# fricker2025-star/Tensor-Cuda-FFT-

Measured on AMD Instinct MI355X. Metric: spectral-mix fwd+bwd GSamples/s (B*N*D/s) at N=4096,D=256; %HBM roofline, higher is better.
Workload: dtype f32

## Files before the change

tensor-cuda-fft-_amd/csrc/smx_core.h:

```cpp
#pragma once
#include <stddef.h>
#include <stdint.h>

#if defined(__HIPCC__)
#include <hip/hip_runtime.h>
#define SMX_HD __host__ __device__ __forceinline__
#else
#define SMX_HD inline
#ifndef __restrict__
#define __restrict__ __restrict
#endif
struct float2 { float x, y; };
#endif

#ifndef SMX_NT_LOAD
#define SMX_NT_LOAD 1
#endif
#ifndef SMX_NT_STORE
#define SMX_NT_STORE 1
#endif

namespace smx {

#if defined(__HIPCC__)
// ... 514 lines not shown
template <int NB, int ROUND>
SMX_HD cf unpack_partner(const TState<NB>& st, const cf* __restrict__ U, int q, int qp, int j, int sl,
                         const ZSave<NB>& zs) {
  constexpr int S0 = ROUND * UnpackRounds<NB>::SLOTS;
  const int ps = partner_slot<NB>(q, sl);
  if (NB >= 4 && (sl & 15) == 0) {
    const bool own_bin = q == 0;
    const int pb = -band_beta(sl >> 4);
    const bool in_range = pb >= -(NB / 2) && pb < NB / 2;
    const cf own = zs.z[in_range ? band_index(pb) : (sl >> 4)];
    const cf u = U[(((own_bin ? sl : ps) - S0) * 16 + qp) * 16 + j];
    return own_bin ? own : u;
  }
  return U[((ps - S0) * 16 + qp) * 16 + j];
}

struct FilterArgs {
  const float* w_re;
  const float* w_im;
  const float* wt;
  const float* bias;
  float* xk_out;
  const float* xk_in;
  float* pslab;
  float* gb_part;
  int conj_w;
  const float* sc;
  float* gsc;
  cf* gsc_part;
  int goff, multi;
  float sp_scale;
  int sp_herm;
};
SMX_HD bool group_edge_slot(const FilterArgs& fa, int fs) {
  return (fa.multi && fs == -512) || (fa.goff > 0 && fs == 0);
}

constexpr int WL_PITCH = 34;
constexpr int WL_ELEMS = 128 * WL_PITCH;
struct WPre { float re[16], im[16]; };
SMX_HD void prefetch_w(WPre& w, const Geom& g, const float* __restrict__ w_re,
                       const float* __restrict__ w_im, int d0, int tid) {
  const int f = tid & 127, h = tid >> 7;
#pragma unroll
  for (int i = 0; i < 16; ++i) {
    const int d = d0 + h + 2 * i;
    const bool ok = d < g.D && f < g.k;
    const size_t o = ok ? (size_t)d * g.F + f : 0;
    const float a = w_re[o], b = w_im[o];
    w.re[i] = ok ? a : 0.f;
    w.im[i] = ok ? b : 0.f;
  }
}
SMX_HD void stage_w(const WPre& w, cf* __restrict__ wl, int tid, int conj_w) {
  const int f = tid & 127, h = tid >> 7;
#pragma unroll
  for (int i = 0; i < 16; ++i) wl[f * WL_PITCH + h + 2 * i] = mk(w.re[i], conj_w ? -w.im[i] : w.im[i]);
}

SMX_HD void synth_pair(const float (&r)[4], bool self, float scale, bool dbl, cf& Spos, cf& Sneg) {
  if (self) {
    Spos = mk(r[0] * scale, r[2] * scale);
    Sneg = Spos;
  } else {
    const float h = dbl ? scale : 0.5f * scale;
    Spos = mk((r[0] - r[3]) * h, (r[1] + r[2]) * h);
    Sneg = mk((r[0] + r[3]) * h, (-r[1] + r[2]) * h);
  }
}
template <int NB>
SMX_HD void synth_fill(TState<NB>& st, const Geom& g, const FilterArgs& fa, int b, int d, bool valid, int q) {
  const int dl = valid ? d : g.D - 2;
  constexpr int CH = NB == 8 ? 16 : 8;
#pragma unroll
  for (int c0 = 0; c0 < 16 * NB; c0 += CH) {
    float r[CH][4];
#pragma unroll
    for (int i = 0; i < CH; ++i) {
      const int fs = slot_fs<NB>(q, c0 + i);
      const int af = fs < 0 ? -fs : fs;
      const int afc = af < g.k ? af : 0;
      ld4(fa.xk_in + (((size_t)b * g.k + afc) * g.D + dl) * 2, r[i][0], r[i][1], r[i][2], r[i][3]);
    }
#pragma unroll
    for (int i = 0; i < CH; ++i) {
      const int fs = slot_fs<NB>(q, c0 + i);
      const int af = fs < 0 ? -fs : fs;
      const bool self = af == 0 || self_nyquist<NB>(g, fs);
      cf sp, sn;
      synth_pair(r[i], self, fa.sp_scale, fa.sp_herm && 2 * af != g.N, sp, sn);
      const cf S = (fs >= 0 || self) ? sp : sn;
      st.acc[c0 + i] = (valid && af < g.k) ? S : mk(0.f, 0.f);
    }
  }
}

template <int NB, int MODE, int ROUND = 0>
SMX_HD void unpack_phase2(TState<NB>& st, const cf* __restrict__ U, const Geom& g,
                          const FilterArgs& fa, int b, int d, bool valid, int q, int j,
                          const ZSave<NB>& zsave = ZSave<NB>{}, const cf* __restrict__ wl = nullptr,
                          cf* gs = nullptr) {
  const int qp = (16 - q) & 15;
  constexpr int S0 = ROUND * UnpackRounds<NB>::SLOTS;
  constexpr int NS = UnpackRounds<NB>::SLOTS;
#ifndef SMX_PF2_FWD
#define SMX_PF2_FWD 4
#endif
#ifndef SMX_PF2_BWD
#define SMX_PF2_BWD 8
#endif
  constexpr int PF = NB == 2 ? (MODE == 1 ? SMX_PF2_BWD : SMX_PF2_FWD) : NB >= 2 ? 4 : 0;
  constexpr bool XQ = MODE == 1 && !io_regs<NB, MODE>() && NB >= 2;
  float wq[PF ? PF : 1][4], xq[PF ? PF : 1][4];
  const int dl = valid ? d : g.D - 2;
  float sca = 1.f, scb = 1.f;
  if (fa.sc) { sca = fa.sc[(size_t)b * g.D + dl]; scb = fa.sc[(size_t)b * g.D + dl + 1]; }
  float gsx = 0.f, gsy = 0.f;
  auto issue = [&](int sl2, int ring) {
    const int fs2 = slot_fs<NB>(q, sl2);
    const int af2 = (fs2 < 0 ? -fs2 : fs2) + fa.goff;
    const int afc = af2 < g.k ? af2 : 0;
    if (MODE != 2) {
      if (fa.wt) {
        ld4(fa.wt + ((size_t)afc * g.D + dl) * 2, wq[ring][0], wq[ring][1], wq[ring][2], wq[ring][3]);
      } else {
        const size_t wo = (size_t)dl * g.F + afc;
        wq[ring][0] = fa.w_re[wo]; wq[ring][1] = fa.w_im[wo];
        wq[ring][2] = fa.w_re[wo + g.F]; wq[ring][3] = fa.w_im[wo + g.F];
      }
    }
    if (XQ && (slot_pos<NB>(sl2) || sl2 == 16 * (NB - 1)))
      ld4(fa.xk_in + (((size_t)b * g.k + afc) * g.D + dl) * 2, xq[ring][0], xq[ring][1], xq[ring][2],
          xq[ring][3]);
  };
  if (PF > 0) {
#pragma unroll
    for (int i = 0; i < PF && i < NS; ++i) issue(S0 + i, i);
  }
#pragma unroll
  for (int sl = S0; sl < S0 + UnpackRounds<NB>::SLOTS; ++sl) {
    const int fs = slot_fs<NB>(q, sl);
    const int af = (fs < 0 ? -fs : fs) + fa.goff;
    const bool snyq = self_nyquist<NB>(g, fs);
    const cf zo = st.acc[sl];
    const cf zp = unpack_partner<NB, ROUND>(st, U, q, qp, j, sl, zsave);
    const int ring = PF ? (sl - S0) % (PF ? PF : 1) : 0;
    float wv[4] = {0.f, 0.f, 0.f, 0.f}, xv[4] = {0.f, 0.f, 0.f, 0.f};
    if (PF > 0) {
#pragma unroll
      for (int c = 0; c < 4; ++c) { wv[c] = wq[ring][c]; xv[c] = xq[ring][c]; }
      if (sl + PF < S0 + NS) issue(sl + PF, ring);
    }
    const cf zpos = fs >= 0 ? zo : zp;
    const cf zneg = fs >= 0 ? zp : zo;
    const cf A = mk(0.5f * (zpos.x + zneg.x), 0.5f * (zpos.y - zneg.y));
    const cf Bc = mk(0.5f * (zpos.y + zneg.y), -0.5f * (zpos.x - zneg.x));
    cf S = mk(0.f, 0.f);
    if (valid && af < g.k && !(NB == 4 && group_edge_slot(fa, fs))) {
      cf wa = mk(0.f, 0.f), wb = mk(0.f, 0.f);
      if (MODE != 2) {
        if (NB == 1 && wl && af < 128) {
          float a0, a1, a2, a3;
          ld4(reinterpret_cast<const float*>(wl + af * WL_PITCH + 2 * j), a0, a1, a2, a3);
          wa = mk(a0, a1); wb = mk(a2, a3);
        } else {
          if (PF > 0) {
            wa = mk(wv[0], wv[1]); wb = mk(wv[2], wv[3]);
          } else if (fa.wt) {
            float a0, a1, a2, a3;
            ld4(fa.wt + ((size_t)af * g.D + d) * 2, a0, a1, a2, a3);
            wa = mk(a0, a1); wb = mk(a2, a3);
          } else {
            const size_t wo = (size_t)d * g.F + af;
            wa = mk(fa.w_re[wo], fa.w_im[wo]);
            wb = mk(fa.w_re[wo + g.F], fa.w_im[wo + g.F]);
          }
          if (fa.conj_w) { wa = cconj(wa); wb = cconj(wb); }
        }
        const cf ya = cscale(cmul(wa, A), sca), yb = cscale(cmul(wb, Bc), scb);
        if (af == 0 || snyq) {
          S = mk(ya.x * g.inv_n, yb.x * g.inv_n);
          if (MODE == 0 && fa.bias && af == 0) S = mk(S.x + fa.bias[d], S.y + fa.bias[d + 1]);
        } else if (fs > 0) {
          S = mk((ya.x - yb.y) * 0.5f * g.inv_n, (ya.y + yb.x) * 0.5f * g.inv_n);
        } else {
          S = mk((ya.x + yb.y) * 0.5f * g.inv_n, (-ya.y + yb.x) * 0.5f * g.inv_n);
        }
      }
      if (fs >= 0 || snyq) {
        const size_t xo = (((size_t)b * g.k + af) * g.D + d) * 2;
        if (io_regs<NB, MODE>() && !snyq) {
          constexpr int IM = io_bins<NB>() - 1;
          if (MODE != 1) {
// ... 103 lines not shown
        ld4(fa.xk_in + xo, xs[i][0], xs[i][1], xs[i][2], xs[i][3]);
      }
    }
#pragma unroll
    for (int i = 0; i < CH; ++i) {
      const int sl = c0 + i;
      const int fs = slot_fs<NB>(q, sl);
      const int af = (fs < 0 ? -fs : fs) + fa.goff;
      const bool ok = valid && af < g.k && !(NB == 4 && group_edge_slot(fa, fs));
      const bool snyq = self_nyquist<NB>(g, fs);
      const bool pos = slot_pos<NB>(sl) || snyq;
      const cf zo = st.acc[sl];
      const cf zpos = fs >= 0 ? zo : zp[i];
      const cf zneg = fs >= 0 ? zp[i] : zo;
      const cf A = mk(0.5f * (zpos.x + zneg.x), 0.5f * (zpos.y - zneg.y));
      const cf Bc = mk(0.5f * (zpos.y + zneg.y), -0.5f * (zpos.x - zneg.x));
      cf S = mk(0.f, 0.f);
      if (MODE != 2) {
        const cf wa = mk(war[i], cj ? -wai[i] : wai[i]);
        const cf wb = mk(wbr[i], cj ? -wbi[i] : wbi[i]);
        const cf ya = cscale(cmul(wa, A), sca), yb = cscale(cmul(wb, Bc), scb);
        const float h = 0.5f * g.inv_n;
        const cf sp = mk((ya.x - yb.y) * h, (ya.y + yb.x) * h);
        const cf sn = mk((ya.x + yb.y) * h, (-ya.y + yb.x) * h);
        cf s0 = mk(ya.x * g.inv_n, yb.x * g.inv_n);
        if (MODE == 0 && fa.bias && af == 0) s0 = mk(s0.x + fa.bias[dl], s0.y + fa.bias[dl + 1]);
        S = (af == 0 || snyq) ? s0 : (fs > 0 ? sp : sn);
        if (!ok) S = mk(0.f, 0.f);
      }
      st.acc[sl] = S;
      if (pos && ok) {
        const size_t xo = (((size_t)b * g.k + af) * g.D + d) * 2;
        if (MODE != 1) {
          if (fa.xk_out) st4(fa.xk_out + xo, A.x, A.y, Bc.x, Bc.y);
        } else {
          const cf pa = cscale(cmulc(mk(xs[i][0], xs[i][1]), A), g.inv_n);
          const cf pb = cscale(cmulc(mk(xs[i][2], xs[i][3]), Bc), g.inv_n);
          {
            const float wai_ = cj ? -wai[i] : wai[i], wbi_ = cj ? -wbi[i] : wbi[i];
            gsx += war[i] * pa.x + wai_ * pa.y; gsy += wbr[i] * pb.x + wbi_ * pb.y;
          }
          st4(fa.pslab + xo, pa.x * sca, pa.y * sca, pb.x * scb, pb.y * scb);
          if (af == 0) {
            fa.gb_part[(size_t)b * g.D + d] = A.x;
            fa.gb_part[(size_t)b * g.D + d + 1] = Bc.x;
          }
        }
      }
    }
  }
  if (MODE == 1 && gs) { gs->x += gsx; gs->y += gsy; }
}

}

namespace smx {

SMX_HD void fwd_phase2_out(const cf* __restrict__ E, const cf* __restrict__ bt_r, int t, int j,
                           cf* __restrict__ dst) {
  cf e[16];
#pragma unroll
  for (int t2 = 0; t2 < 16; ++t2) e[t2] = E[(t2 * 16 + t) * 16 + j];
  fft16<-1>(e);
#pragma unroll
  for (int s = 0; s < 16; ++s) dst[s * TPB] = cmul(ld_uniform(bt_r, s + BT_HALF), e[s]);
}
SMX_HD void inv_phase1_in(cf (&v)[16], const cf* __restrict__ bt_r, cf* __restrict__ E, int q, int j) {
#pragma unroll
  for (int s = 0; s < 16; ++s) v[s] = cmulc(v[s], ld_uniform(bt_r, s + BT_HALF));
  fft16<+1>(v);
#pragma unroll
  for (int p = 0; p < 16; ++p) E[(q * 16 + p) * 16 + j] = v[p];
}

template <int SGN, int L, int STRIDE = 256>
SMX_HD void fft_residues(cf (&a)[L], const cf* __restrict__ tw) {
  if constexpr (L == 8) {
    fft8<SGN>(a);
  } else if constexpr (L == 16) {
    fft16<SGN>(a);
  } else if constexpr (L > 16 && L % 2 == 0) {
    constexpr int H = L / 2;
    cf ev[H], od[H];
#pragma unroll
    for (int i = 0; i < H; ++i) { ev[i] = a[2 * i]; od[i] = a[2 * i + 1]; }
    fft_residues<SGN, H, 2 * STRIDE>(ev, tw);
    fft_residues<SGN, H, 2 * STRIDE>(od, tw);
#pragma unroll
    for (int k = 0; k < H; ++k) {
      const cf w = tw[STRIDE * k];
      const cf o = (SGN < 0) ? cmul(od[k], w) : cmulc(od[k], w);
      a[k] = cadd(ev[k], o);
      a[k + H] = csub(ev[k], o);
    }
  } else if constexpr (L == 4) {
    radix4<SGN>(a[0], a[1], a[2], a[3]);
  } else if constexpr (L == 2) {
    const cf s0 = cadd(a[0], a[1]), d0 = csub(a[0], a[1]);
    a[0] = s0; a[1] = d0;
  } else {
    cf o[L];
#pragma unroll
    for (int f2 = 0; f2 < L; ++f2) {
      cf acc = a[0];
#pragma unroll
      for (int r = 1; r < L; ++r) {
// ... 807 lines not shown
```

tensor-cuda-fft-_amd/csrc/smx_decim.hip:

```cpp
#include "smx_launch.h"

namespace smx {

template <int NB>
__device__ __forceinline__ void zero_acc(TState<NB>& st) {
#pragma unroll
  for (int s = 0; s < 16 * NB; ++s) st.acc[s] = mk(0.f, 0.f);
}

template <int NB, int MODE, bool BATCHED, int ROUND>
__device__ __forceinline__ void unpack_round(TState<NB>& st, cf* lds, const Geom& g,
                                             const FilterArgs& fa, int b, int d, bool valid, int t,
                                             int j, const ZSave<NB>& zs, const WPre* wp, cf* gs) {
  if constexpr (ROUND < UnpackRounds<NB>::N) {
    __syncthreads();
    unpack_phase1<NB, ROUND>(st, lds, t, j);
    const cf* wl = nullptr;
    if constexpr (NB == 1 && MODE != 2) {
      if (wp) { stage_w(*wp, lds + EX, t * 16 + j, fa.conj_w); wl = lds + EX; }
    }
    __syncthreads();
    if constexpr (BATCHED) unpack_phase2_batched<NB, MODE, ROUND>(st, lds, g, fa, b, d, valid, t, j, zs, gs, wl);
    else unpack_phase2<NB, MODE, ROUND>(st, lds, g, fa, b, d, valid, t, j, zs, wl, gs);
    unpack_round<NB, MODE, BATCHED, ROUND + 1>(st, lds, g, fa, b, d, valid, t, j, zs, wp, gs);
  }
}

template <int NB, int MODE, bool BATCHED>
__device__ __forceinline__ void unpack_filter(TState<NB>& st, cf* lds, const Geom& g,
                                              const FilterArgs& fa, int b, int d, bool valid, int t,
                                              int j, const WPre* wp = nullptr) {
  const ZSave<NB> zs = save_z<NB>(st);
  if constexpr (NB == 2 && MODE == 1 && !BATCHED) prefetch_io<NB, MODE>(st, g, fa, b, d, valid, t);
  cf gs = mk(0.f, 0.f);
  const bool want_gs = MODE == 1 && fa.gsc != nullptr;
  unpack_round<NB, MODE, BATCHED, 0>(st, lds, g, fa, b, d, valid, t, j, zs, wp, MODE == 1 ? &gs : nullptr);
  if constexpr (NB == 2 && MODE == 1 && !BATCHED) store_io<NB, MODE>(st, g, fa, b, d, valid, t);
  if constexpr (MODE == 1) {
    if (want_gs) {
      __syncthreads();
      lds[t * 16 + j] = gs;
      __syncthreads();
      if (t == 0 && valid) {
        float sa = 0.f, sb = 0.f;
#pragma unroll
        for (int u = 0; u < 16; ++u) { sa += lds[u * 16 + j].x; sb += lds[u * 16 + j].y; }
        fa.gsc[(size_t)b * g.D + d] = sa;
        fa.gsc[(size_t)b * g.D + d + 1] = sb;
      }
    }
  }
}

struct LnLoad {
  const cf* sb;
  float g0, g1, b0, b1;
};
template <int U0, int CNT>
__device__ __forceinline__ void load_stats(const cf* __restrict__ sb, const Geom& g, int t, int r,
                                           cf (&sv)[16]) {
  const cf* p = sb + (size_t)t * g.L + r;
#pragma unroll
  for (int u = U0; u < U0 + CNT; ++u) sv[u] = p[(size_t)u * 16 * g.L];
}

template <int NB, bool LN, bool DROP, bool PAD, bool LAST, class XB>
__device__ __forceinline__ void forward_tile(TState<NB>& st, cf* E, const XB& xb,
                                             const DecimArgs& a, int t, int j, int r, int rn, cf (&nx)[16],
                                             cf (&ns)[LN ? 16 : 1], const LnLoad* ln, Drop dr, unsigned pj) {
  const Geom& g = a.g;
  if constexpr (LN) {
#pragma unroll
    for (int u = 0; u < 16; ++u)
      st.v[u] = mk(fmaf((nx[u].x - ns[u].x) * ns[u].y, ln->g0, ln->b0),
                   fmaf((nx[u].y - ns[u].x) * ns[u].y, ln->g1, ln->b1));
  } else if constexpr (DROP) {
    const unsigned hd = (unsigned)(g.D >> 1), pstride = 16u * (unsigned)g.L * hd;
    const unsigned p0 = ((unsigned)t * (unsigned)g.L + (unsigned)r) * hd + pj;
#pragma unroll
    for (int u = 0; u < 16; ++u)
      st.v[u] = drop_apply(nx[u], drop_hash(p0 + (unsigned)u * pstride, dr.key), dr.thr, dr.scale);
  } else {
#pragma unroll
    for (int u = 0; u < 16; ++u) st.v[u] = nx[u];
  }
  if constexpr (!LAST) {
    load_rows<0, 8, PAD>(xb, rn, nx);
    if constexpr (LN) load_stats<0, 8>(ln->sb, g, t, rn, ns);
    __builtin_amdgcn_sched_barrier(0);
  }
  fwd_phase1_cp<NB>(st, E, t, j);
  if constexpr (!LAST) load_cp(a.tq + ((size_t)t * g.L + rn) * 16, st.cp);
  __syncthreads();
  if constexpr (!LAST) {
    load_rows<8, 8, PAD>(xb, rn, nx);
    if constexpr (LN) load_stats<8, 8>(ln->sb, g, t, rn, ns);
  }
  fwd_phase2<NB, true>(st, E, a.bt + (size_t)r * BT_STRIDE, t, j);
}

template <int NB, bool LN = false, bool DROP = false, bool PAD = false, class XB>
__device__ __forceinline__ void forward_loop(TState<NB>& st, cf* lds, const XB& xb,
                                             const DecimArgs& a, int t, int j, int rbeg, int cnt,
                                             int rot, const LnLoad* ln = nullptr, Drop dr = Drop{},
                                             unsigned pj = 0) {
  const Geom& g = a.g;
  const int rend = rbeg + cnt;
  cf nx[16];
  cf ns[LN ? 16 : 1];
  int r = rbeg + rot;
  load_rows<0, 16, PAD>(xb, r, nx);
  if constexpr (LN) load_stats<0, 16>(ln->sb, g, t, r, ns);
  load_cp(a.tq + ((size_t)t * g.L + r) * 16, st.cp);
  int i = 0;
  for (; i + 1 < cnt; ++i) {
    int rn = r + 1;
    if (rn == rend) rn = rbeg;
    forward_tile<NB, LN, DROP, PAD, false>(st, lds + (i & 1) * EX, xb, a, t, j, r, rn, nx, ns, ln, dr, pj);
    r = rn;
  }
  forward_tile<NB, LN, DROP, PAD, true>(st, lds + (i & 1) * EX, xb, a, t, j, r, r, nx, ns, ln, dr, pj);
}

template <int NB, bool RES, bool DROP, bool PAD, bool LAST, class YB, class RB>
__device__ __forceinline__ void inverse_tile(TState<NB>& st, cf* E, const YB& yb, const DecimArgs& a,
                                             int t, int j, int r, int rn,
                                             const RB& res, cf (&rx)[RES ? 16 : 1], Drop dr,
                                             unsigned pj, int sw) {
  const Geom& g = a.g;
  inv_phase1<NB, true>(st, a.bt + (size_t)r * BT_STRIDE, E, t, j);
  __syncthreads();
  inv_phase2_gather<NB>(st, E, t, j);
  if constexpr (!LAST) {
    __builtin_amdgcn_sched_barrier(0);
    load_cp(a.tq + ((size_t)t * g.L + rn) * 16, st.cp);
    __builtin_amdgcn_sched_barrier(0);
  }
  fft16<+1>(st.v);
  if constexpr (DROP) {
    const unsigned hd = (unsigned)(g.D >> 1), pstride = 16u * (unsigned)g.L * hd;
    const unsigned p0 = ((unsigned)t * (unsigned)g.L + (unsigned)r) * hd + pj;
#pragma unroll
    for (int u = 0; u < 16; ++u)
      st.v[u] = drop_apply(st.v[u], drop_hash(p0 + (unsigned)u * pstride, dr.key), dr.thr, dr.scale);
  }
  if constexpr (RES) {
#pragma unroll
    for (int u = 0; u < 16; ++u) st.v[u] = cadd(st.v[u], rx[u]);
    if constexpr (!LAST) load_rows<0, 16, PAD>(res, rn, rx);
  }
  store_rows<PAD>(yb, r, st.v, st_tile_mask(a, r, sw));
}

template <int NB, bool RES = false, bool DROP = false, bool PAD = false, class YB, class RB>
__device__ __forceinline__ void inverse_loop(TState<NB>& st, cf* lds, const YB& yb,
                                             const DecimArgs& a, int t, int j, int rbeg,
                                             int cnt, int rot, const RB& res, Drop dr = Drop{},
                                             unsigned pj = 0) {
  const Geom& g = a.g;
  int r = rbeg + rot;
  const int sw = (__builtin_amdgcn_readfirstlane(t) >> 2) >> a.st_wsh;
  cf rx[RES ? 16 : 1];
  if constexpr (RES) load_rows<0, 16, PAD>(res, r, rx);
  load_cp(a.tq + ((size_t)t * g.L + r) * 16, st.cp);
  __builtin_amdgcn_s_waitcnt(0x0F70);
  int i = 0;
  for (; i + 1 < cnt; ++i) {
    int rn = r + 1;
    if (rn == rbeg + cnt) rn = rbeg;
    inverse_tile<NB, RES, DROP, PAD, false>(st, lds + (i & 1) * EX, yb, a, t, j, r, rn, res, rx, dr, pj, sw);
    r = rn;
  }
  inverse_tile<NB, RES, DROP, PAD, true>(st, lds + (i & 1) * EX, yb, a, t, j, r, r, res, rx, dr, pj, sw);
}

__device__ __forceinline__ Drop make_drop(const DecimArgs& a, int b) {
  Drop dr;
  dr.thr = a.drop_thr; dr.scale = a.drop_scale;
  dr.key = drop_row_key(a.rng[0], a.rng[1], b);
  return dr;
}

constexpr bool fused_instance(int nb, int mode, bool drop, bool acc, bool pad, int io, int oio) {
  if (!among<1, 2, 4>::has(nb) || !among<0, 1, 2>::has(mode)) return false;
  if (acc) return nb == 4 && mode != 2 && !drop && io == 0 && oio == 0;
  if (io == 0) return oio == 0 && !(drop && (pad || mode == 2));
  return among<1, 2>::has(io) && mode != 2 && !pad && (oio == io || (oio == 0 && mode == 1));
}
template <int NB, int MODE, bool DROP = false, bool ACC = false, bool PAD = false, int IO = 0, int OIO = IO>
__global__ __launch_bounds__(TPB, 2) void k_fused(const DecimArgs a) {
  SMX_LDS_DECL;
  const Geom& g = a.g;
  const int tid = threadIdx.x, j = tid & 15, t = tid >> 4;
  const int ndt = (g.D + DT - 1) / DT;
  const WgItem w = wg_map(a.bid0 + blockIdx.x, g.B, ndt, 1, g.L, a.placement);
  const int b = w.b, d = w.dt * DT + 2 * j, rot = w.rot;
  const bool valid = d < g.D;
  RowBufT<IO> xb;
  if constexpr (IO == 0) xb = row_buf(a.in + (size_t)b * g.R * g.D, g, t, valid ? d : g.D - 2);
  else xb = row_buf<IO>(a.in, b, g, t, valid ? d : g.D - 2);

  TState<NB> st;
  zero_acc<NB>(st);
  if constexpr (NB == 1) prefetch_io<NB, MODE>(st, g, a.fa, b, d, valid, t);
  WPre wp;
  constexpr bool STAGE_W = NB == 1 && MODE != 2;
  if constexpr (STAGE_W) prefetch_w(wp, g, a.fa.w_re, a.fa.w_im, w.dt * DT, tid);
  Drop dr{};
  if constexpr (DROP) dr = make_drop(a, b);
  const unsigned pj = (unsigned)((valid ? d : g.D - 2) >> 1);
#ifndef SMX_AB_NO_FWD
  forward_loop<NB, false, DROP && MODE == 1, PAD>(st, lds, xb, a, t, j, 0, g.L, rot, nullptr, dr, pj);
#endif
#ifndef SMX_AB_NO_UNPACK
  unpack_filter<NB, MODE, false>(st, lds, g, a.fa, b, d, valid, t, j, STAGE_W ? &wp : nullptr);
#endif
#ifdef SMX_AB_NO_INV
  if (st.acc[0].x == 12345.f) a.out[0] = st.acc[1].y;
  return;
#endif
  if (a.out == nullptr) {
    if constexpr (NB == 1) store_io<NB, MODE>(st, g, a.fa, b, d, valid, t);
    if (a.ws_s != nullptr) {
      cf* s = a.ws_s + (size_t)(b * ndt + w.dt) * (16 * NB * TPB);
#pragma unroll
      for (int sl = 0; sl < 16 * NB; ++sl) s[sl * TPB + tid] = st.acc[sl];
    }
    return;
  }
  __syncthreads();
  RowBufT<OIO> yb;
  if constexpr (OIO == 0) yb = row_buf(a.out + (size_t)b * g.R * g.D, g, t, d, valid);
  else yb = row_buf<OIO>(a.out, b, g, t, d, valid);
  inverse_loop<NB, ACC, DROP && MODE == 0, PAD>(st, lds, yb, a, t, j, 0, g.L, rot, yb, dr, pj);
  if constexpr (NB == 1) store_io<NB, MODE>(st, g, a.fa, b, d, valid, t);
}

template <int NB, bool PAD, bool DROP>
__device__ __forceinline__ void forward16_loop(TState<NB>& st, cf* lds, const float* __restrict__ xb,
                                               const DecimArgs& a, int t, int j, int tbeg, int cnt, int rot,
                                               Drop dr, unsigned pj) {
  const Geom& g = a.g;
  const unsigned hd = (unsigned)(g.D >> 1);
  cf nx[16];
  int tau = tbeg + rot;
  load_tile16<PAD>(xb, g, t, tau, nx);
  cf cn = a.tw[min(16 * tau + t, g.N - 1)];
  for (int i = 0; i < cnt; ++i) {
    if constexpr (DROP) {
      const unsigned p0 = (unsigned)(16 * tau + t) * hd + pj, ps = (unsigned)g.P * hd;
#pragma unroll
      for (int u = 0; u < 16; ++u)
        st.v[u] = drop_apply(nx[u], drop_hash(p0 + (unsigned)u * ps, dr.key), dr.thr, dr.scale);
    } else {
#pragma unroll
      for (int u = 0; u < 16; ++u) st.v[u] = nx[u];
    }
    const cf c = cn;
    int tn = tau + 1;
    if (tn == tbeg + cnt) tn = tbeg;
    if (i + 1 < cnt) {
      load_tile16<PAD>(xb, g, t, tn, nx);
      cn = a.tw[min(16 * tn + t, g.N - 1)];
    }
    cf* E = lds + (i & 1) * EX;
    fwd_phase1<NB>(st, c, E, t, j);
    __syncthreads();
    fwd16_phase2<NB>(st, E, a.v16, a.b16 + (size_t)tau * 32, t, j);
    tau = tn;
  }
}
template <int NB, bool PAD, bool DROP>
__device__ __forceinline__ void inverse16_loop(TState<NB>& st, cf* lds, float* __restrict__ yb, const DecimArgs& a,
                                               int t, int j, bool valid, int tbeg, int cnt, int rot, Drop dr,
                                               unsigned pj) {
  const Geom& g = a.g;
  const unsigned hd = (unsigned)(g.D >> 1);
  int tau = tbeg + rot;
  for (int i = 0; i < cnt; ++i) {
    const cf c = a.tw[min(16 * tau + t, g.N - 1)];
    cf* E = lds + (i & 1) * EX;
    inv16_phase1<NB>(st, a.v16, a.b16 + (size_t)tau * 32, E, t, j);
    __syncthreads();
    inv_phase2<NB>(st, c, E, t, j);
    if constexpr (DROP) {
      const unsigned p0 = (unsigned)(16 * tau + t) * hd + pj, ps = (unsigned)g.P * hd;
#pragma unroll
      for (int u = 0; u < 16; ++u)
        st.v[u] = drop_apply(st.v[u], drop_hash(p0 + (unsigned)u * ps, dr.key), dr.thr, dr.scale);
    }
    store_tile16<PAD>(yb, g, t, tau, valid, st.v);
    ++tau;
    if (tau == tbeg + cnt) tau = tbeg;
  }
}

constexpr bool fused16_instance(int nb, int mode, bool pad, bool drop) {
  return among<1, 2>::has(nb) && among<0, 1, 2>::has(mode) && !(drop && (pad || mode == 2));
}
template <int NB, int MODE, bool PAD = false, bool DROP = false>
__global__ __launch_bounds__(TPB, 2) void k_fused16(const DecimArgs a) {
  SMX_LDS_DECL;
  const Geom& g = a.g;
  const int tid = threadIdx.x, j = tid & 15, t = tid >> 4;
  const int ndt = (g.D + DT - 1) / DT;
  const int T = g.L;
  const WgItem w = wg_map(a.bid0 + blockIdx.x, g.B, ndt, 1, T, a.placement);
  const int b = w.b, d = w.dt * DT + 2 * j, rot = w.rot;
  const bool valid = d < g.D;
  const float* xb = a.in + (size_t)b * g.R * g.D + (valid ? d : g.D - 2);
  TState<NB> st;
  zero_acc<NB>(st);
  if constexpr (NB == 1) prefetch_io<NB, MODE>(st, g, a.fa, b, d, valid, t);
  WPre wp;
  constexpr bool STAGE_W = NB == 1 && MODE != 2;
  if constexpr (STAGE_W) prefetch_w(wp, g, a.fa.w_re, a.fa.w_im, w.dt * DT, tid);
  Drop dr{};
  if constexpr (DROP) dr = make_drop(a, b);
  const unsigned pj = (unsigned)((valid ? d : g.D - 2) >> 1);
  forward16_loop<NB, PAD, DROP && MODE == 1>(st, lds, xb, a, t, j, 0, T, rot, dr, pj);
  unpack_filter<NB, MODE, false>(st, lds, g, a.fa, b, d, valid, t, j, STAGE_W ? &wp : nullptr);
  if (a.out == nullptr) {
    if constexpr (NB == 1) store_io<NB, MODE>(st, g, a.fa, b, d, valid, t);
    if (a.ws_s != nullptr) {
      cf* sp = a.ws_s + (size_t)(b * ndt + w.dt) * (16 * NB * TPB);
#pragma unroll
      for (int sl = 0; sl < 16 * NB; ++sl) sp[sl * TPB + tid] = st.acc[sl];
    }
    return;
  }
  __syncthreads();
  inverse16_loop<NB, PAD, DROP && MODE == 0>(st, lds, a.out + (size_t)b * g.R * g.D + d, a, t, j, valid, 0, T, rot, dr,
                                             pj);
  if constexpr (NB == 1) store_io<NB, MODE>(st, g, a.fa, b, d, valid, t);
}

constexpr bool split16_instance(int nb, bool pad, bool drop) {
  return among<1, 2>::has(nb) && !(pad && drop);
}
template <int NB, bool PAD = false, bool DROP = false>
__global__ __launch_bounds__(TPB, 2) void k_split16_a(const DecimArgs a) {
  SMX_LDS_DECL;
  const Geom& g = a.g;
  const int tid = threadIdx.x, j = tid & 15, t = tid >> 4;
  const int ndt = (g.D + DT - 1) / DT;
  const WgItem w = wg_map(a.bid0 + blockIdx.x, g.B, ndt, a.nsplit, a.lc, a.placement);
  const int c = w.c, b = w.b, wg = b * ndt + w.dt, d = w.dt * DT + 2 * j;
  const bool valid = d < g.D;
  const int tbeg = c * a.lc, cnt = min(a.lc, g.L - tbeg);
  const float* xb = a.in + (size_t)b * g.R * g.D + (valid ? d : g.D - 2);
  TState<NB> st;
  zero_acc<NB>(st);
  Drop dr{};
  if constexpr (DROP) dr = make_drop(a, b);
  if (cnt > 0)
    forward16_loop<NB, PAD, DROP>(st, lds, xb, a, t, j, tbeg, cnt, w.rot % cnt, dr,
                                  (unsigned)((valid ? d : g.D - 2) >> 1));
  cf* z = a.ws_z + ((size_t)wg * a.nsplit + c) * (16 * NB * TPB);
#pragma unroll
  for (int sl = 0; sl < 16 * NB; ++sl) z[sl * TPB + tid] = st.acc[sl];
}
template <int NB, bool PAD = false, bool DROP = false>
__global__ __launch_bounds__(TPB, 2) void k_split16_b(const DecimArgs a) {
  SMX_LDS_DECL;
  const Geom& g = a.g;
  const int tid = threadIdx.x, j = tid & 15, t = tid >> 4;
  const int ndt = (g.D + DT - 1) / DT;
  const WgItem w = wg_map(a.bid0 + blockIdx.x, g.B, ndt, a.nsplit, a.lc, a.placement);
  const int c = w.c, b = w.b, wg = b * ndt + w.dt, d = w.dt * DT + 2 * j;
  const bool valid = d < g.D;
  const int tbeg = c * a.lc, cnt = min(a.lc, g.L - tbeg);
  if (cnt <= 0) return;
  TState<NB> st;
  const cf* sp = a.ws_s + (size_t)wg * (16 * NB * TPB);
// ... 73 lines not shown

  TState<8> st;
  cf nx[16];
  load_tile<PAD>(xb, g, t, 0, nx);
  cf cn = a.tw[(size_t)t * 8];
  full8_fwd_tiles<0, MODE, PAD>(st, lds, xb, a, t, j, nx, cn);
  residue_fft8<-1>(st);
#ifndef SMX_FULL8_BATCHED
#define SMX_FULL8_BATCHED false
#endif
  unpack_filter<8, MODE, SMX_FULL8_BATCHED>(st, lds, g, a.fa, b, d, valid, t, j);
  if (a.out == nullptr) return;
  __syncthreads();
  residue_fft8<+1>(st);
  full8_inv_tiles<0, PAD>(st, lds, a.out + (size_t)b * g.R * g.D + d, a, t, j, valid);
}

template <bool PAD>
__global__ __launch_bounds__(TPB, 1) void k_synth8(const DecimArgs a) {
  SMX_LDS_DECL;
  const Geom& g = a.g;
  const int tid = threadIdx.x, j = tid & 15, t = tid >> 4;
  const int ndt = (g.D + DT - 1) / DT;
  const WgItem w = wg_map(a.bid0 + blockIdx.x, g.B, ndt, 1, g.L, a.placement);
  const int b = w.b, d = w.dt * DT + 2 * j;
  const bool valid = d < g.D;
  TState<8> st;
  synth_fill<8>(st, g, a.fa, b, d, valid, t);
  residue_fft8<+1>(st);
  full8_inv_tiles<0, PAD>(st, lds, a.out + (size_t)b * g.R * g.D + d, a, t, j, valid);
}

template <int NB, bool DROP = false, int IO = 0>
__global__ __launch_bounds__(TPB, NB > 2 ? 1 : 2) void k_fused_blk(const DecimArgs a) {
  SMX_LDS_DECL;
  const Geom& g = a.g;
  const int tid = threadIdx.x, j = tid & 15, t = tid >> 4;
  const int ndt = (g.D + DT - 1) / DT;
  const WgItem w = wg_map(a.bid0 + blockIdx.x, g.B, ndt, 1, g.L, a.placement);
  const int b = w.b, d = w.dt * DT + 2 * j, rot = w.rot;
  const bool valid = d < g.D;
  const int dc = valid ? d : g.D - 2;
  RowBufT<IO> xb;
  if constexpr (IO == 0) xb = row_buf(a.in + (size_t)b * g.R * g.D, g, t, dc);
  else xb = row_buf<IO>(a.in, b, g, t, dc);
  LnLoad ln;
  ln.sb = a.ln_stats + (size_t)b * g.N;
  ln.g0 = a.ln_w ? a.ln_w[dc] : 1.f; ln.g1 = a.ln_w ? a.ln_w[dc + 1] : 1.f;
  ln.b0 = a.ln_b ? a.ln_b[dc] : 0.f; ln.b1 = a.ln_b ? a.ln_b[dc + 1] : 0.f;

  TState<NB> st;
  zero_acc<NB>(st);
  WPre wp;
  if constexpr (NB == 1) prefetch_w(wp, g, a.fa.w_re, a.fa.w_im, w.dt * DT, tid);
  forward_loop<NB, true>(st, lds, xb, a, t, j, 0, g.L, rot, &ln);
  unpack_filter<NB, 0, false>(st, lds, g, a.fa, b, d, valid, t, j, NB == 1 ? &wp : nullptr);
  __syncthreads();
  RowBufT<IO> yb;
  if constexpr (IO == 0) yb = row_buf(a.out + (size_t)b * g.R * g.D, g, t, d, valid);
  else yb = row_buf<IO>(a.out, b, g, t, d, valid);
  Drop dr{};
  if constexpr (DROP) dr = make_drop(a, b);
  inverse_loop<NB, true, DROP>(st, lds, yb, a, t, j, 0, g.L, rot, xb, dr, (unsigned)(dc >> 1));
  if constexpr (NB == 1) store_io<NB, 0>(st, g, a.fa, b, d, valid, t);
}

constexpr bool split_a_instance(int nb, bool drop, bool pad, int io) {
  return among<1, 2, 4>::has(nb) && among<0, 1, 2>::has(io) && !(pad && (drop || io != 0));
}
template <int NB, bool DROP = false, bool PAD = false, int IO = 0>
__global__ __launch_bounds__(TPB, 2) void k_split_a(const DecimArgs a) {
  SMX_LDS_DECL;
  const Geom& g = a.g;
  const int tid = threadIdx.x, j = tid & 15, t = tid >> 4;
  const int ndt = (g.D + DT - 1) / DT;
  const WgItem w = wg_map(a.bid0 + blockIdx.x, g.B, ndt, a.nsplit, a.lc, a.placement);
  const int c = w.c, b = w.b, wg = b * ndt + w.dt, d = w.dt * DT + 2 * j;
  const bool valid = d < g.D;
  const int rbeg = c * a.lc, cnt = min(a.lc, g.L - rbeg);
  RowBufT<IO> xb;
  if constexpr (IO == 0) xb = row_buf(a.in + (size_t)b * g.R * g.D, g, t, valid ? d : g.D - 2);
  else xb = row_buf<IO>(a.in, b, g, t, valid ? d : g.D - 2);
  const int rot = w.rot % cnt;

  TState<NB> st;
  zero_acc<NB>(st);
  Drop dr{};
  if constexpr (DROP) dr = make_drop(a, b);
  forward_loop<NB, false, DROP, PAD>(st, lds, xb, a, t, j, rbeg, cnt, rot, nullptr, dr,
                                     (unsigned)((valid ? d : g.D - 2) >> 1));
  cf* z = a.ws_z + ((size_t)wg * a.nsplit + c) * (16 * NB * TPB);
#pragma unroll
  for (int sl = 0; sl < 16 * NB; ++sl) z[sl * TPB + tid] = st.acc[sl];
}

template <int NB>
__global__ __launch_bounds__(TPB) void k_split_sum(const DecimArgs a) {
  const int sl = blockIdx.x % (16 * NB), wg = blockIdx.x / (16 * NB), tid = threadIdx.x;
  const cf* z = a.ws_z + (size_t)wg * a.nsplit * (16 * NB * TPB) + sl * TPB + tid;
  cf acc = mk(0.f, 0.f);
  int c = 0;
  for (; c + 8 <= a.nsplit; c += 8) {
    cf v[8];
#pragma unroll
    for (int u = 0; u < 8; ++u) v[u] = z[(size_t)(c + u) * (16 * NB * TPB)];
#pragma unroll
    for (int u = 0; u < 8; ++u) acc = cadd(acc, v[u]);
  }
  for (; c < a.nsplit; ++c) acc = cadd(acc, z[(size_t)c * (16 * NB * TPB)]);
  a.ws_zs[(size_t)wg * (16 * NB * TPB) + sl * TPB + tid] = acc;
}

template <int NB, int MODE>
__global__ __launch_bounds__(TPB, NB > 1 ? 1 : 2) void k_split_f(const DecimArgs a) {
  SMX_LDS_DECL;
  const Geom& g = a.g;
// ... 220 lines not shown
```

Before: 339.4.

## Add staged unpack path for NB=1 and carry twiddle state across phases

```diff
diff --git a/tensor-cuda-fft-_amd/csrc/smx_core.h b/tensor-cuda-fft-_amd/csrc/smx_core.h
--- a/tensor-cuda-fft-_amd/csrc/smx_core.h
+++ b/tensor-cuda-fft-_amd/csrc/smx_core.h
@@ -590,6 +590,10 @@
     w.im[i] = ok ? b : 0.f;
   }
 }
+SMX_HD cf prefetch_bias(const Geom& g, const float* __restrict__ bias, int d, bool valid) {
+  const int dl = valid ? d : g.D - 2;
+  return bias ? mk(bias[dl], bias[dl + 1]) : mk(0.f, 0.f);
+}
 SMX_HD void stage_w(const WPre& w, cf* __restrict__ wl, int tid, int conj_w) {
   const int f = tid & 127, h = tid >> 7;
 #pragma unroll
@@ -633,14 +637,15 @@
   }
 }
 
-template <int NB, int MODE, int ROUND = 0>
+template <int NB, int MODE, int ROUND = 0, int SL0 = ROUND * UnpackRounds<NB>::SLOTS,
+          int SL1 = SL0 + UnpackRounds<NB>::SLOTS>
 SMX_HD void unpack_phase2(TState<NB>& st, const cf* __restrict__ U, const Geom& g,
                           const FilterArgs& fa, int b, int d, bool valid, int q, int j,
                           const ZSave<NB>& zsave = ZSave<NB>{}, const cf* __restrict__ wl = nullptr,
                           cf* gs = nullptr) {
   const int qp = (16 - q) & 15;
-  constexpr int S0 = ROUND * UnpackRounds<NB>::SLOTS;
-  constexpr int NS = UnpackRounds<NB>::SLOTS;
+  constexpr int S0 = SL0;
+  constexpr int NS = SL1 - SL0;
 #ifndef SMX_PF2_FWD
 #define SMX_PF2_FWD 4
 #endif
@@ -676,7 +681,7 @@
     for (int i = 0; i < PF && i < NS; ++i) issue(S0 + i, i);
   }
 #pragma unroll
-  for (int sl = S0; sl < S0 + UnpackRounds<NB>::SLOTS; ++sl) {
+  for (int sl = S0; sl < S0 + NS; ++sl) {
     const int fs = slot_fs<NB>(q, sl);
     const int af = (fs < 0 ? -fs : fs) + fa.goff;
     const bool snyq = self_nyquist<NB>(g, fs);
@@ -886,6 +891,98 @@
   if (MODE == 1 && gs) { gs->x += gsx; gs->y += gsy; }
 }
 
+SMX_HD constexpr bool packed_sums_fused(int sl) { return (sl >= 1 && sl <= 4) || (sl >= 8 && sl <= 12); }
+SMX_HD float rounded(float x) {
+#if defined(__HIP_DEVICE_COMPILE__)
+  asm("" : "+v"(x));
+#endif
+  return x;
+}
+SMX_HD cf packed_sums(bool fused, bool pos, cf ca, cf cb, cf ya, cf yb, float sca, float scb) {
+#if defined(__HIP_DEVICE_COMPILE__)
+  if (fused)
+    return pos ? mk(__builtin_fmaf(-scb, cb.y, ya.x), __builtin_fmaf(sca, ca.y, yb.x))
+               : mk(__builtin_fmaf(scb, cb.y, ya.x), __builtin_fmaf(-sca, ca.y, yb.x));
+#endif
+  (void)fused; (void)ca; (void)cb; (void)sca; (void)scb;
+  const float yax = rounded(ya.x), yay = rounded(ya.y), ybx = rounded(yb.x), yby = rounded(yb.y);
+  return pos ? mk(yax - yby, yay + ybx) : mk(yax + yby, -yay + ybx);
+}
+
+template <int MODE>
+SMX_HD void unpack_phase2_staged(TState<1>& st, const cf* __restrict__ U, const Geom& g, const FilterArgs& fa,
+                                 int b, int d, bool valid, int q, int j, const cf* __restrict__ wl, cf bias,
+                                 cf* gs = nullptr) {
+  static_assert(MODE == 0 || MODE == 1, "the spectrum-only launches read no filter");
+  const int qp = (16 - q) & 15;
+  const int dl = valid ? d : g.D - 2;
+  const ZSave<1> zs{};
+  float sca = 1.f, scb = 1.f;
+  if (fa.sc) { sca = fa.sc[(size_t)b * g.D + dl]; scb = fa.sc[(size_t)b * g.D + dl + 1]; }
+  const bool add_bias = MODE == 0 && fa.bias != nullptr;
+  const cf z8 = st.acc[8];
+  cf zp[16];
+  float w[16][4];
+#pragma unroll
+  for (int sl = 0; sl < 16; ++sl) {
+    const int fs = slot_fs<1>(q, sl);
+    const int af = fs < 0 ? -fs : fs;
+    const int afc = (af < g.k && af < 128) ? af : 0;
+    zp[sl] = unpack_partner<1, 0>(st, U, q, qp, j, sl, zs);
+    ld4(reinterpret_cast<const float*>(wl + afc * WL_PITCH + 2 * j), w[sl][0], w[sl][1], w[sl][2], w[sl][3]);
+  }
+  float gsx = 0.f, gsy = 0.f;
+  cf A0 = mk(0.f, 0.f), B0 = mk(0.f, 0.f);
+#pragma unroll
+  for (int sl = 0; sl < 16; ++sl) {
+    const bool pos = sl < 8;
+    const int fs = slot_fs<1>(q, sl);
+    const int af = fs < 0 ? -fs : fs;
+    const bool ok = valid && af < g.k && af < 128;
+    const cf zo = st.acc[sl];
+    const cf zpos = pos ? zo : zp[sl];
+    const cf zneg = pos ? zp[sl] : zo;
+    const cf A = mk(0.5f * (zpos.x + zneg.x), 0.5f * (zpos.y - zneg.y));
+    const cf Bc = mk(0.5f * (zpos.y + zneg.y), -0.5f * (zpos.x - zneg.x));
+    const cf wa = mk(w[sl][0], w[sl][1]), wb = mk(w[sl][2], w[sl][3]);
+    const cf ca = cmul(wa, A), cb = cmul(wb, Bc);
+    const cf ya = cscale(ca, sca), yb = cscale(cb, scb);
+    const cf ps = packed_sums(packed_sums_fused(sl), pos, ca, cb, ya, yb, sca, scb);
+    cf S = mk(ps.x * 0.5f * g.inv_n, ps.y * 0.5f * g.inv_n);
+    if (sl == 0) {
+      cf s0 = mk(rounded(ya.x * g.inv_n), rounded(yb.x * g.inv_n));
+      const cf s0b = mk(s0.x + bias.x, s0.y + bias.y);
+      s0 = add_bias ? s0b : s0;
+      S = af == 0 ? s0 : S;
+      A0 = A; B0 = Bc;
+    }
+    st.acc[sl] = ok ? S : mk(0.f, 0.f);
+    if (pos) {
+      cf& ia = st.io[2 * sl];
+      cf& ib = st.io[2 * sl + 1];
+      if (MODE == 0) {
+        ia = ok ? A : ia; ib = ok ? Bc : ib;
+      } else {
+        const cf pa = cscale(cmulc(ia, A), g.inv_n);
+        const cf pb = cscale(cmulc(ib, Bc), g.inv_n);
+        const float tx = wa.x * pa.x + wa.y * pa.y, ty = wb.x * pb.x + wb.y * pb.y;
+        gsx = ok ? gsx + tx : gsx; gsy = ok ? gsy + ty : gsy;
+        const cf oa = cscale(pa, sca), ob = cscale(pb, scb);
+        ia = ok ? oa : ia; ib = ok ? ob : ib;
+      }
+    }
+  }
+  if (MODE == 1 && q == 0 && valid && g.k > 0) {
+    fa.gb_part[(size_t)b * g.D + d] = A0.x;
+    fa.gb_part[(size_t)b * g.D + d + 1] = B0.x;
+  }
+  if (MODE == 1 && gs) { gs->x += gsx; gs->y += gsy; }
+  if (g.k > 128) {
+    st.acc[8] = z8;
+    unpack_phase2<1, MODE, 0, 8, 9>(st, U, g, fa, b, d, valid, q, j, zs, wl, gs);
+  }
+}
+
 }
 
 namespace smx {
diff --git a/tensor-cuda-fft-_amd/csrc/smx_decim.hip b/tensor-cuda-fft-_amd/csrc/smx_decim.hip
--- a/tensor-cuda-fft-_amd/csrc/smx_decim.hip
+++ b/tensor-cuda-fft-_amd/csrc/smx_decim.hip
@@ -1,6 +1,10 @@
 #include "smx_launch.h"
 
 namespace smx {
+
+#ifndef SMX_CARRY_CP
+#define SMX_CARRY_CP true
+#endif
 
 template <int NB>
 __device__ __forceinline__ void zero_acc(TState<NB>& st) {
@@ -11,7 +15,7 @@
 template <int NB, int MODE, bool BATCHED, int ROUND>
 __device__ __forceinline__ void unpack_round(TState<NB>& st, cf* lds, const Geom& g,
                                              const FilterArgs& fa, int b, int d, bool valid, int t,
-                                             int j, const ZSave<NB>& zs, const WPre* wp, cf* gs) {
+                                             int j, const ZSave<NB>& zs, const WPre* wp, cf bias, cf* gs) {
   if constexpr (ROUND < UnpackRounds<NB>::N) {
     __syncthreads();
     unpack_phase1<NB, ROUND>(st, lds, t, j);
@@ -20,21 +24,28 @@
       if (wp) { stage_w(*wp, lds + EX, t * 16 + j, fa.conj_w); wl = lds + EX; }
     }
     __syncthreads();
+#ifdef SMX_AB_UNPACK_SLOTS
+    constexpr bool STAGED = false;
+#else
+    constexpr bool STAGED = NB == 1 && MODE != 2 && !BATCHED;
+#endif
     if constexpr (BATCHED) unpack_phase2_batched<NB, MODE, ROUND>(st, lds, g, fa, b, d, valid, t, j, zs, gs, wl);
+    else if constexpr (STAGED)
+      unpack_phase2_staged<MODE>(st, lds, g, fa, b, d, valid, t, j, wl, bias, gs);
     else unpack_phase2<NB, MODE, ROUND>(st, lds, g, fa, b, d, valid, t, j, zs, wl, gs);
-    unpack_round<NB, MODE, BATCHED, ROUND + 1>(st, lds, g, fa, b, d, valid, t, j, zs, wp, gs);
+    unpack_round<NB, MODE, BATCHED, ROUND + 1>(st, lds, g, fa, b, d, valid, t, j, zs, wp, bias, gs);
   }
 }
 
 template <int NB, int MODE, bool BATCHED>
 __device__ __forceinline__ void unpack_filter(TState<NB>& st, cf* lds, const Geom& g,
                                               const FilterArgs& fa, int b, int d, bool valid, int t,
-                                              int j, const WPre* wp = nullptr) {
+                                              int j, const WPre* wp = nullptr, cf bias = mk(0.f, 0.f)) {
   const ZSave<NB> zs = save_z<NB>(st);
   if constexpr (NB == 2 && MODE == 1 && !BATCHED) prefetch_io<NB, MODE>(st, g, fa, b, d, valid, t);
   cf gs = mk(0.f, 0.f);
   const bool want_gs = MODE == 1 && fa.gsc != nullptr;
-  unpack_round<NB, MODE, BATCHED, 0>(st, lds, g, fa, b, d, valid, t, j, zs, wp, MODE == 1 ? &gs : nullptr);
+  unpack_round<NB, MODE, BATCHED, 0>(st, lds, g, fa, b, d, valid, t, j, zs, wp, bias, MODE == 1 ? &gs : nullptr);
   if constexpr (NB == 2 && MODE == 1 && !BATCHED) store_io<NB, MODE>(st, g, fa, b, d, valid, t);
   if constexpr (MODE == 1) {
     if (want_gs) {
@@ -64,7 +75,7 @@
   for (int u = U0; u < U0 + CNT; ++u) sv[u] = p[(size_t)u * 16 * g.L];
 }
 
-template <int NB, bool LN, bool DROP, bool PAD, bool LAST, class XB>
+template <int NB, bool LN, bool DROP, bool PAD, bool LAST, bool CARRY, class XB>
 __device__ __forceinline__ void forward_tile(TState<NB>& st, cf* E, const XB& xb,
                                              const DecimArgs& a, int t, int j, int r, int rn, cf (&nx)[16],
                                              cf (&ns)[LN ? 16 : 1], const LnLoad* ln, Drop dr, unsigned pj) {
@@ -90,7 +101,7 @@
     __builtin_amdgcn_sched_barrier(0);
   }
   fwd_phase1_cp<NB>(st, E, t, j);
-  if constexpr (!LAST) load_cp(a.tq + ((size_t)t * g.L + rn) * 16, st.cp);
+  if constexpr (!LAST || CARRY) load_cp(a.tq + ((size_t)t * g.L + rn) * 16, st.cp);
   __syncthreads();
   if constexpr (!LAST) {
     load_rows<8, 8, PAD>(xb, rn, nx);
@@ -99,7 +110,7 @@
   fwd_phase2<NB, true>(st, E, a.bt + (size_t)r * BT_STRIDE, t, j);
 }
 
-template <int NB, bool LN = false, bool DROP = false, bool PAD = false, class XB>
+template <int NB, bool LN = false, bool DROP = false, bool PAD = false, bool CARRY = false, class XB>
 __device__ __forceinline__ void forward_loop(TState<NB>& st, cf* lds, const XB& xb,
                                              const DecimArgs& a, int t, int j, int rbeg, int cnt,
                                              int rot, const LnLoad* ln = nullptr, Drop dr = Drop{},
@@ -116,10 +127,10 @@
   for (; i + 1 < cnt; ++i) {
     int rn = r + 1;
     if (rn == rend) rn = rbeg;
-    forward_tile<NB, LN, DROP, PAD, false>(st, lds + (i & 1) * EX, xb, a, t, j, r, rn, nx, ns, ln, dr, pj);
+    forward_tile<NB, LN, DROP, PAD, false, false>(st, lds + (i & 1) * EX, xb, a, t, j, r, rn, nx, ns, ln, dr, pj);
     r = rn;
   }
-  forward_tile<NB, LN, DROP, PAD, true>(st, lds + (i & 1) * EX, xb, a, t, j, r, r, nx, ns, ln, dr, pj);
+  forward_tile<NB, LN, DROP, PAD, true, CARRY>(st, lds + (i & 1) * EX, xb, a, t, j, r, rbeg + rot, nx, ns, ln, dr, pj);
 }
 
 template <int NB, bool RES, bool DROP, bool PAD, bool LAST, class YB, class RB>
@@ -152,7 +163,7 @@
   store_rows<PAD>(yb, r, st.v, st_tile_mask(a, r, sw));
 }
 
-template <int NB, bool RES = false, bool DROP = false, bool PAD = false, class YB, class RB>
+template <int NB, bool RES = false, bool DROP = false, bool PAD = false, bool CARRIED = false, class YB, class RB>
 __device__ __forceinline__ void inverse_loop(TState<NB>& st, cf* lds, const YB& yb,
                                              const DecimArgs& a, int t, int j, int rbeg,
                                              int cnt, int rot, const RB& res, Drop dr = Drop{},
@@ -162,7 +173,7 @@
   const int sw = (__builtin_amdgcn_readfirstlane(t) >> 2) >> a.st_wsh;
   cf rx[RES ? 16 : 1];
   if constexpr (RES) load_rows<0, 16, PAD>(res, r, rx);
-  load_cp(a.tq + ((size_t)t * g.L + r) * 16, st.cp);
+  if constexpr (!CARRIED) load_cp(a.tq + ((size_t)t * g.L + r) * 16, st.cp);
   __builtin_amdgcn_s_waitcnt(0x0F70);
   int i = 0;
   for (; i + 1 < cnt; ++i) {
@@ -206,14 +217,17 @@
   WPre wp;
   constexpr bool STAGE_W = NB == 1 && MODE != 2;
   if constexpr (STAGE_W) prefetch_w(wp, g, a.fa.w_re, a.fa.w_im, w.dt * DT, tid);
+  cf bias = mk(0.f, 0.f);
+  if constexpr (STAGE_W && MODE == 0) bias = prefetch_bias(g, a.fa.bias, d, valid);
   Drop dr{};
   if constexpr (DROP) dr = make_drop(a, b);
   const unsigned pj = (unsigned)((valid ? d : g.D - 2) >> 1);
+  constexpr bool CARRY = SMX_CARRY_CP && MODE == 0 && !ACC;
 #ifndef SMX_AB_NO_FWD
-  forward_loop<NB, false, DROP && MODE == 1, PAD>(st, lds, xb, a, t, j, 0, g.L, rot, nullptr, dr, pj);
+  forward_loop<NB, false, DROP && MODE == 1, PAD, CARRY>(st, lds, xb, a, t, j, 0, g.L, rot, nullptr, dr, pj);
 #endif
 #ifndef SMX_AB_NO_UNPACK
-  unpack_filter<NB, MODE, false>(st, lds, g, a.fa, b, d, valid, t, j, STAGE_W ? &wp : nullptr);
+  unpack_filter<NB, MODE, false>(st, lds, g, a.fa, b, d, valid, t, j, STAGE_W ? &wp : nullptr, bias);
 #endif
 #ifdef SMX_AB_NO_INV
   if (st.acc[0].x == 12345.f) a.out[0] = st.acc[1].y;
@@ -232,7 +246,7 @@
   RowBufT<OIO> yb;
   if constexpr (OIO == 0) yb = row_buf(a.out + (size_t)b * g.R * g.D, g, t, d, valid);
   else yb = row_buf<OIO>(a.out, b, g, t, d, valid);
-  inverse_loop<NB, ACC, DROP && MODE == 0, PAD>(st, lds, yb, a, t, j, 0, g.L, rot, yb, dr, pj);
+  inverse_loop<NB, ACC, DROP && MODE == 0, PAD, CARRY>(st, lds, yb, a, t, j, 0, g.L, rot, yb, dr, pj);
   if constexpr (NB == 1) store_io<NB, MODE>(st, g, a.fa, b, d, valid, t);
 }
 
@@ -315,11 +329,13 @@
   WPre wp;
   constexpr bool STAGE_W = NB == 1 && MODE != 2;
   if constexpr (STAGE_W) prefetch_w(wp, g, a.fa.w_re, a.fa.w_im, w.dt * DT, tid);
+  cf bias = mk(0.f, 0.f);
+  if constexpr (STAGE_W && MODE == 0) bias = prefetch_bias(g, a.fa.bias, d, valid);
   Drop dr{};
   if constexpr (DROP) dr = make_drop(a, b);
   const unsigned pj = (unsigned)((valid ? d : g.D - 2) >> 1);
   forward16_loop<NB, PAD, DROP && MODE == 1>(st, lds, xb, a, t, j, 0, T, rot, dr, pj);
-  unpack_filter<NB, MODE, false>(st, lds, g, a.fa, b, d, valid, t, j, STAGE_W ? &wp : nullptr);
+  unpack_filter<NB, MODE, false>(st, lds, g, a.fa, b, d, valid, t, j, STAGE_W ? &wp : nullptr, bias);
   if (a.out == nullptr) {
     if constexpr (NB == 1) store_io<NB, MODE>(st, g, a.fa, b, d, valid, t);
     if (a.ws_s != nullptr) {
@@ -499,16 +515,20 @@
   TState<NB> st;
   zero_acc<NB>(st);
   WPre wp;
-  if constexpr (NB == 1) prefetch_w(wp, g, a.fa.w_re, a.fa.w_im, w.dt * DT, tid);
-  forward_loop<NB, true>(st, lds, xb, a, t, j, 0, g.L, rot, &ln);
-  unpack_filter<NB, 0, false>(st, lds, g, a.fa, b, d, valid, t, j, NB == 1 ? &wp : nullptr);
+  cf bias = mk(0.f, 0.f);
+  if constexpr (NB == 1) {
+    prefetch_w(wp, g, a.fa.w_re, a.fa.w_im, w.dt * DT, tid);
+    bias = prefetch_bias(g, a.fa.bias, d, valid);
+  }
+  forward_loop<NB, true, false, false, SMX_CARRY_CP>(st, lds, xb, a, t, j, 0, g.L, rot, &ln);
+  unpack_filter<NB, 0, false>(st, lds, g, a.fa, b, d, valid, t, j, NB == 1 ? &wp : nullptr, bias);
   __syncthreads();
   RowBufT<IO> yb;
   if constexpr (IO == 0) yb = row_buf(a.out + (size_t)b * g.R * g.D, g, t, d, valid);
   else yb = row_buf<IO>(a.out, b, g, t, d, valid);
   Drop dr{};
   if constexpr (DROP) dr = make_drop(a, b);
-  inverse_loop<NB, true, DROP>(st, lds, yb, a, t, j, 0, g.L, rot, xb, dr, (unsigned)(dc >> 1));
+  inverse_loop<NB, true, DROP, false, SMX_CARRY_CP>(st, lds, yb, a, t, j, 0, g.L, rot, xb, dr, (unsigned)(dc >> 1));
   if constexpr (NB == 1) store_io<NB, 0>(st, g, a.fa, b, d, valid, t);
 }
 
```

Result: no change. 336.7 (-0.8%).
